# mcahny/vps

Measured on NVIDIA H100. Metric: FuseTrack frame pairs/s on synthetic 1024x2048 pairs, higher is better.
Workload: dtype f32 (wgmma: 3 split-f16 products per MAC, fp32 accumulate promoted to RN register sums)

## Files before the change

include/vps_b200.h:

```cpp
#ifndef VPS_B200_H_
#define VPS_B200_H_

#include <stdint.h>

#ifdef __cplusplus
extern "C" {
#endif

#define VPS_OK 0
#define VPS_E_ARG (-1)
#define VPS_E_CUDA (-2)
#define VPS_E_NODEV (-3)

#define VPS_F32 0
#define VPS_BF16 1

#define VPS_ACT_NONE 0
#define VPS_ACT_RELU 1
#define VPS_ACT_LRELU 2
#define VPS_ACT_SIGMOID 3

typedef struct vps_tensor {
  void* ptr;
  int32_t n, h, w, c;
// ... 7 lines not shown
void vps_add_launch_count(int64_t n);

typedef struct vps_conv_args {
  vps_tensor x, y, res;
  const void* w;
  const float* bias;
  int32_t kh, kw, sh, sw, ph, pw;
  int32_t oh, ow;
  int32_t oy_mul, oy_off, ox_mul, ox_off;
  int32_t cin, cout;
  int32_t act;
  float slope;
  int32_t res_after_act;
  float out_scale;
  int32_t cin_gran;
} vps_conv_args;

int vps_conv2d_tc(const vps_conv_args* a, void* stream);
int vps_conv2d_tc_multi(const vps_conv_args* a, int nprob, void* stream);
int vps_conv2d_simt(const vps_conv_args* a, void* stream);
int vps_pack_weights_tc(const float* w_oihw, const float* scale, void* dst_bf16, int cout, int cin,
                        int kh, int kw, int transposed, int cin_gran, void* stream);
int vps_pack_weights_simt(const float* w_oihw, const float* scale, float* dst, int cout, int cin,
                          int kh, int kw, int transposed, void* stream);
int64_t vps_packed_tc_bytes(int cout, int cin, int kh, int kw, int cin_gran);

int vps_conv2d_tc32(const vps_conv_args* a, void* stream);
int vps_conv2d_tc32_multi(const vps_conv_args* a, int nprob, void* stream);
int vps_conv2d_tc32_plan(const vps_conv_args* a, int nprob, int* plan);
int vps_pack_weights_tc32(const float* w_oihw, const float* scale, void* dst, int cout, int cin, int kh, int kw,
                          int transposed, int prob, int nprob, void* stream);
int64_t vps_packed_tc32_bytes(int cout, int cin, int kh, int kw, int nprob);
int vps_tc32_overflow(int reset);
int vps_deform_conv_tc32(const vps_tensor* x, const vps_tensor* offset, const void* w, int cout, const vps_tensor* y,
                         void* stream);
int vps_deform_conv_tc32_plan(const vps_tensor* x, int cout, int* plan);

int vps_im2col(const vps_tensor* x, const vps_tensor* cols, int kh, int kw, int sh, int sw, int ph,
               int pw, void* stream);

int vps_correlation(const vps_tensor* f1, const vps_tensor* f2, const vps_tensor* out, int pad,
                    int max_disp, int stride1, int stride2, int act, float slope, void* stream);
int vps_correlation_tc(const vps_tensor* f1, const vps_tensor* f2, const vps_tensor* out, int pad,
                       int max_disp, int stride1, int stride2, int act, float slope, void* stream);
// ... 112 lines not shown
```

vps_b200/_lib.py:

```python
import ctypes as C
import os

_HERE = os.path.dirname(os.path.abspath(__file__))
LIB_PATH = os.path.join(_HERE, "lib", "libvps_b200.so")

VPS_F32, VPS_BF16 = 0, 1
ACT_NONE, ACT_RELU, ACT_LRELU, ACT_SIGMOID = 0, 1, 2, 3


class VpsTensor(C.Structure):
    _fields_ = [("ptr", C.c_void_p), ("n", C.c_int32), ("h", C.c_int32), ("w", C.c_int32),
                ("c", C.c_int32), ("cs", C.c_int32), ("dtype", C.c_int32)]


class VpsConvArgs(C.Structure):
    _fields_ = [("x", VpsTensor), ("y", VpsTensor), ("res", VpsTensor),
                ("w", C.c_void_p), ("bias", C.c_void_p),
                ("kh", C.c_int32), ("kw", C.c_int32), ("sh", C.c_int32), ("sw", C.c_int32),
                ("ph", C.c_int32), ("pw", C.c_int32),
                ("oh", C.c_int32), ("ow", C.c_int32),
                ("oy_mul", C.c_int32), ("oy_off", C.c_int32), ("ox_mul", C.c_int32), ("ox_off", C.c_int32),
                ("cin", C.c_int32), ("cout", C.c_int32),
                ("act", C.c_int32), ("slope", C.c_float), ("res_after_act", C.c_int32),
                ("out_scale", C.c_float), ("cin_gran", C.c_int32)]


class VpsError(RuntimeError):
    pass


_lib = None


def lib():
    global _lib
    if _lib is None:
        if not os.path.exists(LIB_PATH):
            raise VpsError(
                "libvps_b200.so not found at %s -- run `python -c 'import __graft_entry__ as g; g.build()'`; "
                "there is no CPU/PyTorch fallback for the product path" % LIB_PATH)
        _lib = C.CDLL(LIB_PATH)
        _lib.vps_last_error.restype = C.c_char_p
        _lib.vps_launch_count.restype = C.c_int64
        _lib.vps_packed_tc_bytes.restype = C.c_int64
        _lib.vps_packed_tc32_bytes.restype = C.c_int64
        _lib.vps_correlation_tc32_ws_bytes.restype = C.c_int64
        _lib.vps_unify_pan_ws_bytes.restype = C.c_int64
        _lib.vps_unify_pan_error_offset.restype = C.c_int64
        _lib.vps_tube_confusion_ws_bytes.restype = C.c_int64
        _lib.vps_tube_confusion_ws_bytes.argtypes = [C.c_int64]
        _lib.vps_add_launch_count.restype = None
        _lib.vps_add_launch_count.argtypes = [C.c_int64]
    return _lib


def check(status, what=""):
    if status != 0:
        raise VpsError("%s failed (%d): %s" % (what, status, lib().vps_last_error().decode()))


EXPORTS = [
    "vps_last_error", "vps_version", "vps_launch_count", "vps_add_launch_count",
    "vps_conv2d_tc", "vps_conv2d_tc_multi", "vps_conv2d_simt", "vps_pack_weights_tc", "vps_pack_weights_simt",
    "vps_packed_tc_bytes", "vps_im2col",
    "vps_conv2d_tc32", "vps_conv2d_tc32_multi", "vps_conv2d_tc32_plan", "vps_pack_weights_tc32", "vps_packed_tc32_bytes", "vps_tc32_overflow", "vps_deform_conv_tc32", "vps_deform_conv_tc32_plan",
    "vps_correlation", "vps_correlation_tc", "vps_correlation_simt", "vps_correlation_tc32", "vps_correlation_tc32_ws_bytes", "vps_resample2d", "vps_channelnorm", "vps_flownet_input", "vps_flownet_stage", "vps_flownet_cat3", "vps_flow_deconv",
    "vps_nchw_to_nhwc", "vps_nhwc_to_nchw", "vps_copy_scale", "vps_axpby",
    "vps_space_to_depth2", "vps_tap_gather3x3", "vps_preprocess_u8", "vps_resize_bilinear", "vps_resize_nearest", "vps_pool2d", "vps_groupnorm",
    "vps_bfp_gather", "vps_bfp_scatter", "vps_flow_warp", "vps_tcea_temporal", "vps_tcea_combine",
    "vps_deform_im2col", "vps_deform_conv_tc",
    "vps_roi_align", "vps_sort_desc", "vps_rpn_decode", "vps_nms", "vps_nms_batch", "vps_sigmoid_flat", "vps_gather_rows",
    "vps_maskroi_candidates", "vps_track_assign",
    "vps_rpn_finalize", "vps_maskroi_finalize", "vps_select_class", "vps_track_update", "vps_det_split",
    "vps_mask_removal", "vps_panoptic_fuse", "vps_unify_pan", "vps_unify_pan_ws_bytes", "vps_unify_pan_error", "vps_unify_pan_error_offset", "vps_tube_confusion", "vps_tube_confusion_ws_bytes", "vps_rgb_to_id", "vps_pan2ch_ids",
]
```

vps_b200/csrc/conv_tc32.cu:

```cuda
#include "conv_tc_common.cuh"

namespace {

constexpr int T32_CONV_WARPS = 3;
constexpr int T32_KC = 32;
constexpr int T32_MAX_N = 128;
constexpr int T32_WIDE_MAX_N = 64;
constexpr int t32_threads(int nwg) { return 128 * (nwg + 1); }
constexpr int T32_STAGE_SLOTS = 2;
constexpr int T32_PLANES = 2;

__device__ unsigned int g_tc32_overflow = 0;

struct Tc32Extra {
  int rows;
  int plane_bytes;
  int stage_bytes;
  int b_plane_bytes;
  int dcn;
  int dcn_split_n;
};

struct Dcn32Params {
  const float* x;
  const float* off;
  int x_cs, off_cs, H, W;
};
constexpr int dcn32_setup_bytes(int rows) { return 9 * rows * 32; }
constexpr int DCN32_THREADS = 512;
constexpr int DCN32_GATHER_WARPS = 7;
constexpr int DCN32_MAX_N = 128;
constexpr int DCN32_LO_REGS = 80, DCN32_HI_REGS = 176;
static_assert(128 * (2 * DCN32_LO_REGS + 2 * DCN32_HI_REGS) == DCN32_THREADS * (65536 / DCN32_THREADS),
              "the DCN register split must use exactly the launch allocation");
static_assert(DCN32_LO_REGS % 8 == 0 && DCN32_HI_REGS % 8 == 0 && DCN32_LO_REGS >= 24 && DCN32_HI_REGS <= 256,
// ... 45 lines not shown
          }
          if (++ss == T32_STAGE_SLOTS) { ss = 0; sphase ^= 1; }
        }
        mbar_wait(rg.bempty(bs), bphase ^ 1);
        if (elect_one()) {
          mbar_expect_tx(rg.bfull(bs), b_bytes);
          tma_load_5d(rg.b_base + bs * rg.b_bytes, tmB, rg.bfull(bs), cc * T32_KC, n0, tap, t.prob, 0);
        }
        if (++bs == p.b_stages) { bs = 0; bphase ^= 1; }
        if (++s == kw) { s = 0; ++r; }
      }
    }
  }
}

__device__ __forceinline__ void converter32(const ConvTcParams& p, const Tc32Extra& e, const Ring32& rg, int ctid, int nthreads) {
  const int ntaps = p.kh * p.kw;
  const int items_per_tile = p.cin_chunks * (p.halo ? 1 : ntaps);
  const int tasks = e.rows * 4;
  int ss = 0, as = 0;
  uint32_t sphase = 0, aphase = 0;
  bool over = false;
  for (int tile = blockIdx.x; tile < p.total_tiles; tile += gridDim.x) {
    for (int it = 0; it < items_per_tile; ++it) {
      mbar_wait(rg.sfull(ss), sphase);
      mbar_wait(rg.pempty(as), aphase ^ 1);
      const uint32_t src = rg.s_base + ss * rg.s_bytes;
      const uint32_t dst = rg.a_base + as * rg.a_bytes;
      for (int task = ctid; task < tasks; task += nthreads) {
        const int r = task >> 2, j = task & 3;
// ... 265 lines not shown
template <int NWG, bool TMA_EPI>
__global__ void __launch_bounds__(t32_threads(NWG), 1)
conv_igemm_tc32_kernel(const __grid_constant__ CUtensorMap tmA, const __grid_constant__ CUtensorMap tmB,
                       const __grid_constant__ CUtensorMap tmY, const __grid_constant__ CUtensorMap tmR, const ConvTcParams p,
                       const Tc32Extra e) {
  extern __shared__ __align__(1024) uint8_t smem_raw[];
  const uint32_t smem_base = (smem_u32(smem_raw) + 1023u) & ~1023u;
  Ring32 rg;
  rg.s_base = smem_base; rg.s_bytes = (uint32_t)e.stage_bytes;
  rg.a_base = rg.s_base + T32_STAGE_SLOTS * rg.s_bytes; rg.a_bytes = (uint32_t)T32_PLANES * (uint32_t)e.plane_bytes;
  rg.b_base = rg.a_base + (uint32_t)p.a_stages * rg.a_bytes; rg.b_bytes = (uint32_t)T32_PLANES * (uint32_t)e.b_plane_bytes;
  rg.e_base = rg.b_base + (uint32_t)p.b_stages * rg.b_bytes;
  rg.bias_base = rg.e_base + (TMA_EPI ? 64u * NWG * (uint32_t)p.block_n * 4u : 0u);
  rg.bar_base = rg.bias_base + (TMA_EPI ? (uint32_t)NWG * (uint32_t)p.block_n * 4u : 0u);
  const int warp = __shfl_sync(0xffffffffu, (int)threadIdx.x >> 5, 0);
  if (warp == 0) init_bars32(rg, 32 * T32_CONV_WARPS, 32 * T32_CONV_WARPS, NWG);
  if (threadIdx.x == 32) {
    asm volatile("prefetch.tensormap [%0];" ::"l"(&tmA) : "memory");
    asm volatile("prefetch.tensormap [%0];" ::"l"(&tmB) : "memory");
    if (TMA_EPI) {
      asm volatile("prefetch.tensormap [%0];" ::"l"(&tmY) : "memory");
      if (p.res) asm volatile("prefetch.tensormap [%0];" ::"l"(&tmR) : "memory");
    }
  }
  __syncthreads();
  asm volatile("griddepcontrol.wait;" ::: "memory");
  asm volatile("griddepcontrol.launch_dependents;" ::: "memory");
  if (warp == 0) producer32(p, e, rg, &tmA, &tmB);
  else if (warp < 4) converter32(p, e, rg, (int)threadIdx.x - 32, 32 * T32_CONV_WARPS);
  else consumer32_n<NWG, TMA_EPI>(p, e, rg, (warp - 4) >> 2, &tmY, &tmR);
}

__global__ void __launch_bounds__(DCN32_THREADS, 1)
dcn_igemm_tc32_kernel(const __grid_constant__ CUtensorMap tmB, const ConvTcParams p, const Tc32Extra e, const Dcn32Params d) {
  extern __shared__ __align__(1024) uint8_t smem_raw[];
  const uint32_t smem_base = (smem_u32(smem_raw) + 1023u) & ~1023u;
  Ring32 rg;
  rg.s_base = smem_base; rg.s_bytes = 0;
  rg.a_base = smem_base; rg.a_bytes = (uint32_t)T32_PLANES * (uint32_t)e.plane_bytes;
  rg.b_base = rg.a_base + (uint32_t)p.a_stages * rg.a_bytes; rg.b_bytes = (uint32_t)T32_PLANES * (uint32_t)e.b_plane_bytes;
  const uint32_t setup_base = rg.b_base + (uint32_t)p.b_stages * rg.b_bytes;
  rg.bar_base = setup_base + dcn32_setup_bytes(e.rows);
  const int warp = __shfl_sync(0xffffffffu, (int)threadIdx.x >> 5, 0);
  if (warp == 0) init_bars32(rg, (uint32_t)e.rows / 8u, 1, 2);
// ... 24 lines not shown
                                         unsigned short* __restrict__ bl, int cout, int cin, int kh, int kw, int cout_pad,
                                         int cin_pad, int transposed) {
  const int64_t total = (int64_t)cout_pad * kh * kw * cin_pad;
  bool over = false;
  for (int64_t i = blockIdx.x * (int64_t)blockDim.x + threadIdx.x; i < total; i += (int64_t)gridDim.x * blockDim.x) {
    const float v = packed_weight(src, scale, i, cout, cin, kh, kw, cin_pad, transposed);
    unsigned short h, l;
    split_f16(v, h, l);
    over = over || f16_over(v);
    bm[i] = h;
    bl[i] = l;
  }
  if (over) atomicAdd(&g_tc32_overflow, 1u);
}

inline int64_t plane_elems(int cout, int cin, int kh, int kw) {
  const int64_t cout_pad = (cout + 15) / 16 * 16, cin_pad = (cin + T32_KC - 1) / T32_KC * T32_KC;
  return cout_pad * kh * kw * cin_pad;
}

constexpr int T32_SMEM_BUDGET = 227 * 1024 - 1024 - T32_BAR_BYTES - 64;

struct Tc32Plan {
  int nwg;
  int block_n;
  int halo, tw, th, halo_w, halo_h;
  int rows, stage_bytes, plane_bytes, a_stages, a_side;
  int b_stages;
  int epi_tma;
};

bool tc32_epi_expressible(const vps_conv_args* a, int nprob) {
  if (nprob != 1 || a->oy_mul != 1 || a->ox_mul != 1 || a->y.dtype != VPS_F32) return false;
  const int64_t px = (int64_t)a->oy_off * a->y.w + a->ox_off;
  if ((((uintptr_t)a->y.ptr + px * a->y.cs * 4) & 15) || a->y.cs % 4) return false;
  if (a->res.ptr && (a->res.dtype != VPS_F32 || (((uintptr_t)a->res.ptr + px * a->res.cs * 4) & 15) || a->res.cs % 4))
    return false;
  return true;
}

Tc32Plan tc32_tile(const vps_conv_args* a, int nwg) {
  Tc32Plan g = {};
  g.nwg = nwg;
  const int px = 64 * nwg;
  g.halo = a->sh == 1 && a->sw == 1 && a->kh * a->kw > 1 && a->kh <= 8 && a->kw <= 8;
  g.tw = g.halo ? 8 : patch_tw(a->oh, a->ow, px, a->sh, a->sw);
  g.th = px / g.tw;
  g.halo_w = g.tw + a->kw - 1;
  g.halo_h = g.th + a->kh - 1;
  g.rows = g.halo ? g.halo_h * g.halo_w : px;
  g.stage_bytes = (g.rows * 128 + 1023) / 1024 * 1024;
  g.plane_bytes = (g.rows * 64 + 1023) / 1024 * 1024;
  g.a_stages = g.halo ? 2 : 3;
  g.a_side = T32_STAGE_SLOTS * g.stage_bytes + g.a_stages * T32_PLANES * g.plane_bytes;
  return g;
}

int tc32_plan(const vps_conv_args* a, int nprob, Tc32Plan& out) {
  VPS_CHECK_ARG(nprob >= 1 && nprob <= MAX_PROB, "conv2d_tc32: nprob %d", nprob);
  VPS_CHECK_ARG(a->sh >= 1 && a->sh <= 2 && a->sw >= 1 && a->sw <= 2, "conv2d_tc32: stride must be 1 or 2");
  VPS_CHECK_ARG(a->kh >= 1 && a->kw >= 1 && a->cin >= 1 && a->cout >= 1 && a->oh >= 0 && a->ow >= 0 && a->x.n >= 0,
                "conv2d_tc32: bad geometry (k %dx%d, cin %d, cout %d, out %dx%d)", a->kh, a->kw, a->cin, a->cout, a->oh, a->ow);
  const int sms = vps::num_sms();
  if (sms <= 0) { vps::set_error("no device"); return VPS_E_NODEV; }
  const int cout_pad = (a->cout + 15) / 16 * 16;
  const int steps = (a->cin + T32_KC - 1) / T32_KC * a->kh * a->kw;
  double best = -1.0;
  for (int nwg = 2; nwg <= 4; nwg += 2) {
    Tc32Plan g = tc32_tile(a, nwg);
    const int64_t m_tiles = (int64_t)a->x.n * vps::cdiv(a->oh, g.th) * vps::cdiv(a->ow, g.tw) * nprob;
// ... 4 lines not shown
      const int64_t tiles = m_tiles * (cout_pad / bn);
      const double waves = (double)((tiles + sms - 1) / sms);
      const double step = fmax(fmax(300.0, 1.5 * nwg * bn), fmax((double)(bn * 64 * T32_PLANES) / 56.0, conv));
      const double t = waves * ((double)steps * step + 40.0 * bn + 1500.0);
      if (best < 0 || t < best * 0.999) {
        best = t;
        out = g;
        out.block_n = bn;
      }
    }
  }
  if (best < 0) {
    vps::set_error("conv2d_tc32: ring does not fit (k %dx%d)", a->kh, a->kw);
    return VPS_E_ARG;
  }
  const int eb = t32_epi_bytes(out.nwg, out.block_n), b2 = 2 * T32_PLANES * out.block_n * 64;
  out.epi_tma = 0;
  if (!out.halo && out.block_n <= T32_EPI_MAX_N && tc32_epi_expressible(a, nprob)) {
    if (out.a_side + b2 + eb > T32_SMEM_BUDGET && out.a_stages == 3 &&
        out.a_side - T32_PLANES * out.plane_bytes + b2 + eb <= T32_SMEM_BUDGET) {
      out.a_stages = 2;
      out.a_side -= T32_PLANES * out.plane_bytes;
    }
    out.epi_tma = out.a_side + b2 + eb <= T32_SMEM_BUDGET;
  }
  const int bst = (T32_SMEM_BUDGET - out.a_side - (out.epi_tma ? eb : 0)) / (T32_PLANES * out.block_n * 64);
  out.b_stages = bst > MAX_STAGES ? MAX_STAGES : bst;
  return VPS_OK;
}

// ... 40 lines not shown
    }
  }
  if (best < 0) {
    vps::set_error("deform_conv_tc32: no tiling fits (cout %d)", cout);
    return VPS_E_ARG;
  }
  return VPS_OK;
}

}

extern "C" int64_t vps_packed_tc32_bytes(int cout, int cin, int kh, int kw, int nprob) {
  return plane_elems(cout, cin, kh, kw) * 2 * T32_PLANES * nprob;
}

extern "C" unsigned int* vps_tc32_overflow_flag() {
  unsigned int* p = nullptr;
  if (cudaGetSymbolAddress((void**)&p, g_tc32_overflow) != cudaSuccess) return nullptr;
  return p;
}

extern "C" int vps_tc32_overflow(int reset) {
  unsigned int v = 0;
  if (cudaMemcpyFromSymbol(&v, g_tc32_overflow, sizeof(v)) != cudaSuccess) return -1;
  if (reset && v) {
    const unsigned int z = 0;
    cudaMemcpyToSymbol(g_tc32_overflow, &z, sizeof(z));
  }
  return (int)v;
}

extern "C" int vps_pack_weights_tc32(const float* w, const float* scale, void* dst, int cout, int cin, int kh, int kw,
                                     int transposed, int prob, int nprob, void* stream) {
  VPS_CHECK_ARG(nprob >= 1 && nprob <= MAX_PROB && prob >= 0 && prob < nprob, "pack_weights_tc32: prob %d of %d", prob, nprob);
// ... 28 lines not shown
  if (st != VPS_OK) return st;
  VPS_CHECK_ARG(g.b_stages >= 2, "conv2d_tc32: ring does not fit (%d x %d px halo, bn %d)", g.halo_h, g.halo_w, g.block_n);
  ConvTcParams p = {};
  Tc32Extra e = {};
  p.bk = T32_KC;
  const int cin_pad = (a->cin + T32_KC - 1) / T32_KC * T32_KC;
  const int cout_pad = (a->cout + 15) / 16 * 16;
  p.n_img = a->x.n; p.oh = a->oh; p.ow = a->ow;
  const bool halo = g.halo != 0;
  p.halo = g.halo;
  p.tw = g.tw; p.th = g.th;
  p.halo_w = g.halo_w;
  const int halo_h = g.halo_h;
  e.rows = g.rows;
  p.a_box_bytes = e.rows * 128;
  e.stage_bytes = g.stage_bytes;
  e.plane_bytes = g.plane_bytes;
  p.a_stage_bytes = T32_PLANES * e.plane_bytes;
  p.tiles_x = vps::cdiv(a->ow, p.tw); p.tiles_y = vps::cdiv(a->oh, p.th);
  p.kh = a->kh; p.kw = a->kw; p.sh = a->sh; p.sw = a->sw;
  p.cin_chunks = cin_pad / T32_KC;
  const int rem = a->cin - (p.cin_chunks - 1) * T32_KC;
  p.nk_last = (rem + 15) / 16;
  const int ntaps = a->kh * a->kw;
  p.a_stages = g.a_stages;
  const int block_n = g.block_n;
  p.block_n = block_n; p.n_tiles_n = cout_pad / block_n;
  e.b_plane_bytes = block_n * 64;
  p.b_stages = g.b_stages;
  p.nprob = nprob;
  p.tiles_per_prob = p.n_img * p.tiles_y * p.tiles_x * p.n_tiles_n;
  p.total_tiles = p.tiles_per_prob * nprob;
  st = set_problems(p, args, nprob, "conv2d_tc32");
  if (st != VPS_OK) return st;
  if (p.total_tiles == 0) return VPS_OK;

  CUtensorMap tmA, tmB;
  if (!vps::encode_nhwc(&tmA, a->x, CU_TENSOR_MAP_DATA_TYPE_FLOAT32, T32_KC, halo ? p.halo_w : p.tw * a->sw,
                        halo ? halo_h : p.th * a->sh, a->sw, a->sh, CU_TENSOR_MAP_SWIZZLE_128B, CU_TENSOR_MAP_L2_PROMOTION_L2_128B,
                        "conv2d_tc32: encode A"))
    return VPS_E_CUDA;
  const int64_t n_plane = (int64_t)cout_pad * ntaps * cin_pad;
  {
    cuuint64_t dims[5] = {(cuuint64_t)cin_pad, (cuuint64_t)cout_pad, (cuuint64_t)ntaps, (cuuint64_t)nprob, T32_PLANES};
    cuuint64_t strides[4] = {(cuuint64_t)ntaps * cin_pad * 2, (cuuint64_t)cin_pad * 2, (cuuint64_t)n_plane * 2,
                             (cuuint64_t)n_plane * nprob * 2};
    cuuint32_t box[5] = {(cuuint32_t)T32_KC, (cuuint32_t)block_n, 1, 1, T32_PLANES};
    cuuint32_t estr[5] = {1, 1, 1, 1, 1};
    CUresult r = encode(&tmB, CU_TENSOR_MAP_DATA_TYPE_UINT16, 5, (void*)a->w, dims, strides, box, estr, CU_TENSOR_MAP_INTERLEAVE_NONE,
                        CU_TENSOR_MAP_SWIZZLE_64B, CU_TENSOR_MAP_L2_PROMOTION_L2_256B, CU_TENSOR_MAP_FLOAT_OOB_FILL_NONE);
    if (r != CUDA_SUCCESS) { vps::set_error("conv2d_tc32: encode B failed (%d)", (int)r); return VPS_E_CUDA; }
  }
  CUtensorMap tmY = {}, tmR = {};
  if (g.epi_tma) {
    const int bc = t32_box_c(block_n), box_w = p.tw < 64 ? p.tw : 64;
    const int64_t px = (int64_t)a->oy_off * a->y.w + a->ox_off;
    for (int m = 0; m < (a->res.ptr ? 2 : 1); ++m) {
      const vps_tensor& t = m ? a->res : a->y;
      vps_tensor v = t;
      v.ptr = (float*)t.ptr + px * t.cs; v.n = a->x.n; v.h = a->oh; v.w = a->ow; v.c = a->cout;
      if (!vps::encode_nhwc(m ? &tmR : &tmY, v, CU_TENSOR_MAP_DATA_TYPE_FLOAT32, bc, box_w, 64 / box_w, 1, 1,
                            bc == 32 ? CU_TENSOR_MAP_SWIZZLE_128B : CU_TENSOR_MAP_SWIZZLE_64B, CU_TENSOR_MAP_L2_PROMOTION_L2_128B,
                            m ? "conv2d_tc32: encode residual" : "conv2d_tc32: encode output", &t))
        return VPS_E_CUDA;
    }
  }
  const int smem = g.a_side + p.b_stages * T32_PLANES * e.b_plane_bytes + (g.epi_tma ? t32_epi_bytes(g.nwg, block_n) : 0) + 1024 +
                   T32_BAR_BYTES;
#define VPS_TC32_LAUNCH(NWG, EPI)                                                                                              \
  launch_persistent<conv_igemm_tc32_kernel<NWG, EPI>>(p.total_tiles, t32_threads(NWG), smem, stream, "conv2d_tc32", tmA, tmB, tmY, \
                                                      tmR, p, e)
  if (g.nwg == 4) return g.epi_tma ? VPS_TC32_LAUNCH(4, true) : VPS_TC32_LAUNCH(4, false);
  return g.epi_tma ? VPS_TC32_LAUNCH(2, true) : VPS_TC32_LAUNCH(2, false);
#undef VPS_TC32_LAUNCH
}

extern "C" int vps_conv2d_tc32(const vps_conv_args* a, void* stream) { return vps_conv2d_tc32_multi(a, 1, stream); }

extern "C" int vps_conv2d_tc32_plan(const vps_conv_args* a, int nprob, int* plan) {
  Tc32Plan g;
  const int st = tc32_plan(a, nprob, g);
  if (st != VPS_OK) return st;
  plan[0] = g.nwg; plan[1] = g.block_n; plan[2] = g.tw; plan[3] = g.th; plan[4] = g.halo; plan[5] = g.epi_tma;
  return VPS_OK;
}


extern "C" int vps_deform_conv_tc32(const vps_tensor* x, const vps_tensor* offset, const void* w, int cout, const vps_tensor* y,
                                    void* stream) {
  VPS_CHECK_ARG(x->dtype == VPS_F32 && offset->dtype == VPS_F32 && offset->c >= 18, "deform_conv_tc32: dtypes");
  VPS_CHECK_ARG(x->c % T32_KC == 0 && x->cs % 8 == 0 && ((uintptr_t)x->ptr & 31) == 0,
                "deform_conv_tc32: x must have cin %% 32 == 0 and 32-byte aligned pixel rows (256-bit sampling loads)");
  VPS_CHECK_ARG(offset->n == x->n && offset->h == x->h && offset->w == x->w && y->n == x->n && y->h == x->h && y->w == x->w &&
                    y->c == cout, "deform_conv_tc32: shapes");
  VPS_CHECK_ARG((int64_t)x->n * x->h * x->w * x->cs < (1ll << 31), "deform_conv_tc32: tensor too large for 32-bit offsets");
  VPS_CHECK_ARG(((uintptr_t)w & 127) == 0, "deform_conv_tc32: weights not aligned");
  auto encode = vps::tensor_map_encoder();
  if (!encode) return VPS_E_CUDA;
  VPS_CHECK_ARG(y->dtype == VPS_F32, "deform_conv_tc32: y must be fp32");
// ... 56 lines not shown
```

vps_b200/csrc/corr_tc.cu:

```cuda
#include "conv_tc_common.cuh"

namespace {

constexpr int NPIX = 96;
constexpr int KC = 64;
constexpr int A_BYTES = 128 * KC * 2;
constexpr int B_BYTES = NPIX * KC * 2;
constexpr int A_STAGES = 6;
constexpr int MAX_KCH = 4;

struct CorrParams {
  int H, W, C, kch;
  int tiles_x, tiles_y, total_tiles;
  int n_img;
  void* out; int out_cs, out_dtype;
  int act; float slope;
  float scale;
  int accumulate;
  int f16;
};

template <int R, int S2, bool F16>
__device__ __forceinline__ void corr_consumer(const CorrParams& p, uint32_t a_ring, uint32_t b_buf, uint32_t bars, int wg) {
  constexpr int D = 2 * R + 1;
// ... 149 lines not shown
  static bool attr_set = false;
  if (!attr_set) {
    if (cudaFuncSetAttribute(kern, cudaFuncAttributeMaxDynamicSharedMemorySize, smem) != cudaSuccess) {
      vps::set_error("correlation_tc: smem attr: %s", cudaGetErrorString(cudaGetLastError()));
      return VPS_E_CUDA;
    }
    attr_set = true;
  }
  const int sms = vps::num_sms();
  const int grid = p.total_tiles < sms ? p.total_tiles : sms;
  kern<<<grid, 384, smem, st>>>(tm1, tm2, p);
  VPS_CUDA_LAST("corr_tc_kernel");
  return VPS_OK;
}

__global__ void split_f16_planes_kernel(const float* __restrict__ x, int64_t npix, int c, int cs, __half* __restrict__ hi,
                                        __half* __restrict__ lo, unsigned int* overflow) {
  const int64_t total = npix * (c / 4);
  bool over = false;
  for (int64_t i = blockIdx.x * (int64_t)blockDim.x + threadIdx.x; i < total; i += (int64_t)gridDim.x * blockDim.x) {
    const int64_t pix = i / (c / 4);
    const int c4 = (int)(i - pix * (c / 4)) * 4;
    const float4 v = *reinterpret_cast<const float4*>(x + pix * cs + c4);
    const float vv[4] = {v.x, v.y, v.z, v.w};
    __half h[4], l[4];
#pragma unroll
    for (int k = 0; k < 4; ++k) {
      unsigned short hb, lb;
      split_f16(vv[k], hb, lb);
      over = over || f16_over(vv[k]);
      h[k] = __ushort_as_half(hb); l[k] = __ushort_as_half(lb);
    }
    *reinterpret_cast<uint2*>(hi + pix * c + c4) = *reinterpret_cast<const uint2*>(h);
    *reinterpret_cast<uint2*>(lo + pix * c + c4) = *reinterpret_cast<const uint2*>(l);
  }
  if (over && overflow) atomicAdd(overflow, 1u);
}

}

extern "C" unsigned int* vps_tc32_overflow_flag();

extern "C" int64_t vps_correlation_tc32_ws_bytes(const vps_tensor* f1) {
  return 4 * (int64_t)f1->n * f1->h * f1->w * f1->c * 2 + 1024;
}

extern "C" int vps_correlation_tc32(const vps_tensor* f1, const vps_tensor* f2, const vps_tensor* out, int pad, int max_disp,
                                    int stride1, int stride2, int act, float slope, void* ws, void* stream) {
  VPS_CHECK_ARG(stride1 == 1 && pad == max_disp, "correlation_tc32: only stride1=1, pad==max_displacement");
  VPS_CHECK_ARG(f1->dtype == VPS_F32 && f2->dtype == VPS_F32 && out->dtype == VPS_F32, "correlation_tc32: fp32 tensors only");
  VPS_CHECK_ARG(f1->h == f2->h && f1->w == f2->w && f1->c == f2->c && f1->n == f2->n && out->h == f1->h && out->w == f1->w,
                "correlation_tc32: shape mismatch");
  VPS_CHECK_ARG(f1->c % KC == 0 && f1->c <= KC * MAX_KCH, "correlation_tc32: C must be a multiple of 64, <= 256");
  VPS_CHECK_ARG(f1->cs % 4 == 0 && f2->cs % 4 == 0 && ((uintptr_t)f1->ptr & 15) == 0 && ((uintptr_t)f2->ptr & 15) == 0 &&
                    ws && ((uintptr_t)ws & 255) == 0, "correlation_tc32: features / scratch must be aligned");
  VPS_CHECK_ARG(act == VPS_ACT_NONE || act == VPS_ACT_LRELU, "correlation_tc32: act");
  const int R = max_disp / stride2, D = 2 * R + 1;
  VPS_CHECK_ARG(out->c == D * D, "correlation_tc32: out.c %d != %d", out->c, D * D);
  VPS_CHECK_ARG((R == 10 && stride2 == 2) || (R == 4 && stride2 == 1), "correlation_tc32: unsupported (max_disp %d, stride2 %d)",
                max_disp, stride2);
  cudaStream_t st = (cudaStream_t)stream;
  const int64_t npix = (int64_t)f1->n * f1->h * f1->w, plane = npix * f1->c;
  __half* base = (__half*)ws;
  vps_tensor t[4];
  for (int i = 0; i < 4; ++i) {
    t[i] = *f1; t[i].ptr = base + i * plane; t[i].cs = f1->c; t[i].dtype = VPS_BF16;
  }
  unsigned int* flag = vps_tc32_overflow_flag();
  const int blocks = (int)((npix * (f1->c / 4) + 255) / 256 > 8192 ? 8192 : (npix * (f1->c / 4) + 255) / 256);
  split_f16_planes_kernel<<<blocks, 256, 0, st>>>((const float*)f1->ptr, npix, f1->c, f1->cs, base, base + plane, flag);
  VPS_CUDA_LAST("split_f16_planes");
  split_f16_planes_kernel<<<blocks, 256, 0, st>>>((const float*)f2->ptr, npix, f1->c, f2->cs, base + 2 * plane, base + 3 * plane, flag);
  VPS_CUDA_LAST("split_f16_planes");
  const float s1 = 1.0f / (float)f1->c, s2 = s1 * T32_LO_INV;
  int rc;
#define CORR_PASS(A, B, SC, ACC, ACT)                                                                        \
  rc = (R == 10) ? launch<10, 2>(&t[A], &t[B], out, ACT, slope, st, SC, ACC, 1) : launch<4, 1>(&t[A], &t[B], out, ACT, slope, st, SC, ACC, 1); \
  if (rc != VPS_OK) return rc;
  CORR_PASS(0, 2, s1, 0, VPS_ACT_NONE)
  CORR_PASS(0, 3, s2, 1, VPS_ACT_NONE)
  CORR_PASS(1, 2, s2, 1, act)
#undef CORR_PASS
  return VPS_OK;
}

extern "C" int vps_correlation_tc(const vps_tensor* f1, const vps_tensor* f2, const vps_tensor* out, int pad, int max_disp,
                                  int stride1, int stride2, int act, float slope, void* stream) {
  VPS_CHECK_ARG(stride1 == 1 && pad == max_disp, "correlation_tc: only stride1=1, pad==max_displacement");
  VPS_CHECK_ARG(f1->dtype == VPS_BF16 && f2->dtype == VPS_BF16, "correlation_tc: bf16 features only");
  VPS_CHECK_ARG(f1->h == f2->h && f1->w == f2->w && f1->c == f2->c && f1->n == f2->n && out->h == f1->h && out->w == f1->w,
// ... 14 lines not shown
```

vps_b200/ops.py:

```python
import ctypes as C
import os

import torch

from . import _lib
from ._lib import (ACT_LRELU, ACT_NONE, ACT_RELU, ACT_SIGMOID, VPS_BF16, VPS_F32, VpsConvArgs, VpsError,
                   VpsTensor, check, lib)

_DT = {torch.float32: VPS_F32, torch.bfloat16: VPS_BF16}

PROFILE = None
_NOTE = {"flops": 0, "tag": ""}
SCOPE = [""]
_real_lib = lib


class _ProfLib(object):
    def __getattr__(self, name):
        f = getattr(_real_lib(), name)
        if PROFILE is None or not name.startswith("vps_") or name in ("vps_last_error", "vps_launch_count", "vps_packed_tc_bytes"):
            return f

        def w(*a):
            s, e = torch.cuda.Event(enable_timing=True), torch.cuda.Event(enable_timing=True)
# ... 160 lines not shown
    kh, kw = pw.kh, pw.kw
    sh, sw = (stride, stride) if isinstance(stride, int) else stride
    ph, pw_ = pad_hw if pad_hw is not None else ((pad, pad) if isinstance(pad, int) else pad)
    a.kh, a.kw, a.sh, a.sw, a.ph, a.pw = kh, kw, sh, sw, ph, pw_
    if oh is None:
        oh = (x.shape[1] + 2 * ph - kh) // sh + 1
        ow = (x.shape[2] + 2 * pw_ - kw) // sw + 1
    a.oh, a.ow = oh, ow
    a.oy_mul, a.oy_off, a.ox_mul, a.ox_off = omap
    a.cin, a.cout = pw.cin, pw.cout
    a.act, a.slope, a.res_after_act, a.out_scale = act, slope, int(res_after_act), out_scale
    a.bias = pw.bias.data_ptr() if pw.bias is not None else None
    return a


def conv2d(x, pw, y, stride=1, pad=0, act=ACT_NONE, slope=0.1, res=None, res_after_act=False, out_scale=1.0,
           oh=None, ow=None, omap=(1, 0, 1, 0), pad_hw=None, use_tc=None):
    a = _conv_args(x, pw, y, stride, pad, act, slope, res, res_after_act, out_scale, oh, ow, omap, pad_hw)
    if use_tc is None:
        use_tc = x.dtype == torch.bfloat16
    if PROFILE is not None:
        _NOTE["flops"] = _NOTE.pop("flops_alg", None) or 2 * x.shape[0] * a.oh * a.ow * pw.cout * pw.cin * a.kh * a.kw
        _NOTE["tag"] = "%dx%d s%d %d->%d @%dx%d" % (a.kh, a.kw, a.sh, pw.cin, pw.cout, a.oh, a.ow)
    if use_tc and x.dtype == torch.float32:
        a.w = pw.tc32().data_ptr()
        check(lib().vps_conv2d_tc32(C.byref(a), stream()), "conv2d_tc32")
    elif use_tc:
        a.cin_gran = pw.gran()
        a.w = pw.tc().data_ptr()
        check(lib().vps_conv2d_tc(C.byref(a), stream()), "conv2d_tc")
    else:
        a.w = pw.simt().data_ptr()
        check(lib().vps_conv2d_simt(C.byref(a), stream()), "conv2d_simt")
    return y


def conv2d_tc_multi(x, pws, y, pads, omaps, act=ACT_NONE, slope=0.1, out_scale=1.0, oh=None, ow=None, shared32=None):
    n = len(pws)
    arr = (VpsConvArgs * n)()
    gran = pws[0].gran()
    f32 = x.dtype == torch.float32
    for i in range(n):
        a = _conv_args(x, pws[i], y, 1, 0, act, slope, None, False, out_scale, oh, ow, omaps[i], pads[i])
        a.cin_gran = gran
        a.w = shared32.data_ptr() if f32 else pws[i].tc(gran).data_ptr()
        arr[i] = a
    if PROFILE is not None:
        _NOTE["flops"] = 2 * x.shape[0] * arr[0].oh * arr[0].ow * pws[0].cout * pws[0].cin * arr[0].kh * arr[0].kw * n
        _NOTE["tag"] = "%dx%d x%d phases %d->%d @%dx%d" % (arr[0].kh, arr[0].kw, n, pws[0].cin, pws[0].cout, arr[0].oh, arr[0].ow)
    if f32:
        check(lib().vps_conv2d_tc32_multi(arr, n, stream()), "conv2d_tc32_multi")
    else:
        check(lib().vps_conv2d_tc_multi(arr, n, stream()), "conv2d_tc_multi")
    return y


def conv2d_tc32_plan(x, pws, stride=1, pad=0, oh=None, ow=None, pads=None, y=None, res=None, omaps=None):
    pws = pws if isinstance(pws, (list, tuple)) else [pws]
    n = len(pws)
    arr = (VpsConvArgs * n)()
    for i in range(n):
        arr[i] = _conv_args(x, pws[i], x if y is None else y, stride, pad, ACT_NONE, 0.1, res, False, 1.0, oh, ow,
                            omaps[i] if omaps is not None else (1, 0, 1, 0), pads[i] if pads is not None else None)
    plan = (C.c_int * 6)()
    check(_real_lib().vps_conv2d_tc32_plan(arr, n, plan), "conv2d_tc32_plan")
    return dict(nwg=plan[0], block_n=plan[1], tw=plan[2], th=plan[3], halo=plan[4], epilogue="tma" if plan[5] else "frag")


def correlation(f1, f2, out, pad, max_disp, stride1, stride2, act=ACT_NONE, slope=0.1, impl=None):
    fn = {None: "vps_correlation", "tc": "vps_correlation_tc", "simt": "vps_correlation_simt", "tc32": "vps_correlation_tc32"}[impl]
    if PROFILE is not None:
        d = 2 * (max_disp // stride2) + 1
        _NOTE["flops"] = 2 * f1.shape[0] * f1.shape[1] * f1.shape[2] * f1.shape[3] * d * d
        _NOTE["tag"] = "corr d%d s%d C%d @%dx%d" % (max_disp, stride2, f1.shape[3], f1.shape[1], f1.shape[2])
    if impl is None and F32_TC[0] and f1.dtype == torch.float32 and f2.dtype == torch.float32 and out.dtype == torch.float32:
        c = f1.shape[3]
        if (c % 64 == 0 and c <= 256 and stride1 == 1 and pad == max_disp and (max_disp, stride2) == (20, 2)
                and vt(f1).cs % 4 == 0 and vt(f2).cs % 4 == 0 and f1.data_ptr() % 16 == 0 and f2.data_ptr() % 16 == 0):
            fn = "vps_correlation_tc32"
    if fn == "vps_correlation_tc32":
        ws = torch.empty(int(lib().vps_correlation_tc32_ws_bytes(C.byref(vt(f1)))), dtype=torch.uint8, device=f1.device)
# ... 274 lines not shown
```

Before: 16.57.

## Add pre-split f16 feed path for tc32 convolutions chosen by cost model

Adds an optional feed mode for the fp32 tensor-core convolution. The input is split once into f16 hi/lo planes in a workspace by a separate kernel, and the producer then TMA-loads those planes directly, so the converter warps are bypassed. An auto cost model enables this when per-element conversion work inside the kernel, repeated across taps and N tiles, outweighs one extra split pass. The exchange is an extra kernel launch, workspace allocation and extra HBM traffic. The split kernel is now shared with correlation.

```diff
diff --git a/include/vps_b200.h b/include/vps_b200.h
--- a/include/vps_b200.h
+++ b/include/vps_b200.h
@@ -45,7 +45,12 @@
   int32_t res_after_act;
   float out_scale;
   int32_t cin_gran;
+  int32_t feed;
+  void* ws;
 } vps_conv_args;
+#define VPS_TC32_FEED_AUTO 0
+#define VPS_TC32_FEED_CONVERT 1
+#define VPS_TC32_FEED_PRESPLIT 2
 
 int vps_conv2d_tc(const vps_conv_args* a, void* stream);
 int vps_conv2d_tc_multi(const vps_conv_args* a, int nprob, void* stream);
@@ -59,6 +64,7 @@
 int vps_conv2d_tc32(const vps_conv_args* a, void* stream);
 int vps_conv2d_tc32_multi(const vps_conv_args* a, int nprob, void* stream);
 int vps_conv2d_tc32_plan(const vps_conv_args* a, int nprob, int* plan);
+int64_t vps_conv2d_tc32_ws_bytes(const vps_conv_args* a, int nprob);
 int vps_pack_weights_tc32(const float* w_oihw, const float* scale, void* dst, int cout, int cin, int kh, int kw,
                           int transposed, int prob, int nprob, void* stream);
 int64_t vps_packed_tc32_bytes(int cout, int cin, int kh, int kw, int nprob);
diff --git a/vps_b200/_lib.py b/vps_b200/_lib.py
--- a/vps_b200/_lib.py
+++ b/vps_b200/_lib.py
@@ -22,7 +22,10 @@
                 ("oy_mul", C.c_int32), ("oy_off", C.c_int32), ("ox_mul", C.c_int32), ("ox_off", C.c_int32),
                 ("cin", C.c_int32), ("cout", C.c_int32),
                 ("act", C.c_int32), ("slope", C.c_float), ("res_after_act", C.c_int32),
-                ("out_scale", C.c_float), ("cin_gran", C.c_int32)]
+                ("out_scale", C.c_float), ("cin_gran", C.c_int32), ("feed", C.c_int32), ("ws", C.c_void_p)]
+
+
+TC32_FEED = {None: 0, "convert": 1, "presplit": 2}
 
 
 class VpsError(RuntimeError):
@@ -45,6 +48,7 @@
         _lib.vps_packed_tc_bytes.restype = C.c_int64
         _lib.vps_packed_tc32_bytes.restype = C.c_int64
         _lib.vps_correlation_tc32_ws_bytes.restype = C.c_int64
+        _lib.vps_conv2d_tc32_ws_bytes.restype = C.c_int64
         _lib.vps_unify_pan_ws_bytes.restype = C.c_int64
         _lib.vps_unify_pan_error_offset.restype = C.c_int64
         _lib.vps_tube_confusion_ws_bytes.restype = C.c_int64
@@ -63,7 +67,7 @@
     "vps_last_error", "vps_version", "vps_launch_count", "vps_add_launch_count",
     "vps_conv2d_tc", "vps_conv2d_tc_multi", "vps_conv2d_simt", "vps_pack_weights_tc", "vps_pack_weights_simt",
     "vps_packed_tc_bytes", "vps_im2col",
-    "vps_conv2d_tc32", "vps_conv2d_tc32_multi", "vps_conv2d_tc32_plan", "vps_pack_weights_tc32", "vps_packed_tc32_bytes", "vps_tc32_overflow", "vps_deform_conv_tc32", "vps_deform_conv_tc32_plan",
+    "vps_conv2d_tc32", "vps_conv2d_tc32_multi", "vps_conv2d_tc32_plan", "vps_conv2d_tc32_ws_bytes", "vps_pack_weights_tc32", "vps_packed_tc32_bytes", "vps_tc32_overflow", "vps_deform_conv_tc32", "vps_deform_conv_tc32_plan",
     "vps_correlation", "vps_correlation_tc", "vps_correlation_simt", "vps_correlation_tc32", "vps_correlation_tc32_ws_bytes", "vps_resample2d", "vps_channelnorm", "vps_flownet_input", "vps_flownet_stage", "vps_flownet_cat3", "vps_flow_deconv",
     "vps_nchw_to_nhwc", "vps_nhwc_to_nchw", "vps_copy_scale", "vps_axpby",
     "vps_space_to_depth2", "vps_tap_gather3x3", "vps_preprocess_u8", "vps_resize_bilinear", "vps_resize_nearest", "vps_pool2d", "vps_groupnorm",
diff --git a/vps_b200/csrc/conv_tc32.cu b/vps_b200/csrc/conv_tc32.cu
--- a/vps_b200/csrc/conv_tc32.cu
+++ b/vps_b200/csrc/conv_tc32.cu
@@ -19,6 +19,7 @@
   int b_plane_bytes;
   int dcn;
   int dcn_split_n;
+  int presplit;
 };
 
 struct Dcn32Params {
@@ -94,6 +95,38 @@
   }
 }
 
+__device__ __forceinline__ void producer32_presplit(const ConvTcParams& p, const Ring32& rg, const CUtensorMap* tmA,
+                                                    const CUtensorMap* tmB, uint32_t b_bytes) {
+  const int ntaps = p.kh * p.kw, kw = p.kw;
+  const uint32_t a_box_bytes = (uint32_t)p.a_box_bytes;
+  int as = 0, bs = 0;
+  uint32_t aphase = 0, bphase = 0;
+  for (int tile = blockIdx.x; tile < p.total_tiles; tile += gridDim.x) {
+    const TileCoord t = tile_coord(p, tile);
+    const int x_base = t.tx * p.tw * p.sw - p.pw_[t.prob];
+    const int y_base = t.ty * p.th * p.sh - p.ph_[t.prob];
+    const int n0 = t.n_idx * p.block_n;
+    for (int cc = 0; cc < p.cin_chunks; ++cc) {
+      int r = 0, s = 0;
+      for (int tap = 0; tap < ntaps; ++tap) {
+        mbar_wait(rg.pempty(as), aphase ^ 1);
+        if (elect_one()) {
+          mbar_expect_tx(rg.pfull(as), a_box_bytes);
+          tma_load_5d(rg.a_base + as * rg.a_bytes, tmA, rg.pfull(as), cc * T32_KC, x_base + s, y_base + r, t.img, 0);
+        }
+        if (++as == p.a_stages) { as = 0; aphase ^= 1; }
+        mbar_wait(rg.bempty(bs), bphase ^ 1);
+        if (elect_one()) {
+          mbar_expect_tx(rg.bfull(bs), b_bytes);
+          tma_load_5d(rg.b_base + bs * rg.b_bytes, tmB, rg.bfull(bs), cc * T32_KC, n0, tap, t.prob, 0);
+        }
+        if (++bs == p.b_stages) { bs = 0; bphase ^= 1; }
+        if (++s == kw) { s = 0; ++r; }
+      }
+    }
+  }
+}
+
 __device__ __forceinline__ void converter32(const ConvTcParams& p, const Tc32Extra& e, const Ring32& rg, int ctid, int nthreads) {
   const int ntaps = p.kh * p.kw;
   const int items_per_tile = p.cin_chunks * (p.halo ? 1 : ntaps);
@@ -389,7 +422,7 @@
   rg.bias_base = rg.e_base + (TMA_EPI ? 64u * NWG * (uint32_t)p.block_n * 4u : 0u);
   rg.bar_base = rg.bias_base + (TMA_EPI ? (uint32_t)NWG * (uint32_t)p.block_n * 4u : 0u);
   const int warp = __shfl_sync(0xffffffffu, (int)threadIdx.x >> 5, 0);
-  if (warp == 0) init_bars32(rg, 32 * T32_CONV_WARPS, 32 * T32_CONV_WARPS, NWG);
+  if (warp == 0) init_bars32(rg, e.presplit ? 1 : 32 * T32_CONV_WARPS, 32 * T32_CONV_WARPS, NWG);
   if (threadIdx.x == 32) {
     asm volatile("prefetch.tensormap [%0];" ::"l"(&tmA) : "memory");
     asm volatile("prefetch.tensormap [%0];" ::"l"(&tmB) : "memory");
@@ -401,8 +434,11 @@
   __syncthreads();
   asm volatile("griddepcontrol.wait;" ::: "memory");
   asm volatile("griddepcontrol.launch_dependents;" ::: "memory");
-  if (warp == 0) producer32(p, e, rg, &tmA, &tmB);
-  else if (warp < 4) converter32(p, e, rg, (int)threadIdx.x - 32, 32 * T32_CONV_WARPS);
+  if (warp == 0 && e.presplit) producer32_presplit(p, rg, &tmA, &tmB, (uint32_t)T32_PLANES * (uint32_t)e.b_plane_bytes);
+  else if (warp == 0) producer32(p, e, rg, &tmA, &tmB);
+  else if (warp < 4) {
+    if (!e.presplit) converter32(p, e, rg, (int)threadIdx.x - 32, 32 * T32_CONV_WARPS);
+  }
   else consumer32_n<NWG, TMA_EPI>(p, e, rg, (warp - 4) >> 2, &tmY, &tmR);
 }
 
@@ -457,6 +493,37 @@
   if (over) atomicAdd(&g_tc32_overflow, 1u);
 }
 
+__global__ void split_f16_planes_kernel(const float* __restrict__ x, int64_t npix, int c, int cs, int c_pad,
+                                        uint4* __restrict__ hi, uint4* __restrict__ lo) {
+  const int chunks = c_pad / 8;
+  const int64_t total = npix * chunks;
+  bool over = false;
+  for (int64_t i = blockIdx.x * (int64_t)blockDim.x + threadIdx.x; i < total; i += (int64_t)gridDim.x * blockDim.x) {
+    const int64_t pix = i / chunks;
+    const int c0 = (int)(i - pix * chunks) * 8;
+    const float* src = x + pix * cs + c0;
+    float v[8];
+#pragma unroll
+    for (int q = 0; q < 2; ++q) {
+      if (c0 + 4 * q + 4 <= c) {
+        const float4 f = *reinterpret_cast<const float4*>(src + 4 * q);
+        v[4 * q] = f.x; v[4 * q + 1] = f.y; v[4 * q + 2] = f.z; v[4 * q + 3] = f.w;
+      } else {
+#pragma unroll
+        for (int k = 0; k < 4; ++k) v[4 * q + k] = c0 + 4 * q + k < c ? src[4 * q + k] : 0.f;
+      }
+    }
+    uint4 h, l;
+    split_pair_f16(v[0], v[1], h.x, l.x, over);
+    split_pair_f16(v[2], v[3], h.y, l.y, over);
+    split_pair_f16(v[4], v[5], h.z, l.z, over);
+    split_pair_f16(v[6], v[7], h.w, l.w, over);
+    hi[i] = h;
+    lo[i] = l;
+  }
+  if (over) atomicAdd(&g_tc32_overflow, 1u);
+}
+
 inline int64_t plane_elems(int cout, int cin, int kh, int kw) {
   const int64_t cout_pad = (cout + 15) / 16 * 16, cin_pad = (cin + T32_KC - 1) / T32_KC * T32_KC;
   return cout_pad * kh * kw * cin_pad;
@@ -471,6 +538,7 @@
   int rows, stage_bytes, plane_bytes, a_stages, a_side;
   int b_stages;
   int epi_tma;
+  int presplit;
 };
 
 bool tc32_epi_expressible(const vps_conv_args* a, int nprob) {
@@ -497,6 +565,39 @@
   g.a_stages = g.halo ? 2 : 3;
   g.a_side = T32_STAGE_SLOTS * g.stage_bytes + g.a_stages * T32_PLANES * g.plane_bytes;
   return g;
+}
+
+constexpr double T32_CONV_ITEM_CLK = 2000.0, T32_CONV_ROW_CLK = 6.0;
+constexpr double T32_FED_STEP_CLK = 950.0, T32_FED_MMA_CLK = 5.25;
+constexpr double T32_SPLIT_BYTES_PER_CLK = 1300.0;
+constexpr int T32_PRESPLIT_MIN_REUSE = 8;
+
+bool tc32_presplit_pays(const vps_conv_args* a, int nprob, const Tc32Plan& g, int sms) {
+  if (g.halo || nprob != 1 || a->oh == 0 || a->ow == 0 || a->kh < a->sh || a->kw < a->sw) return false;
+  if ((a->oh - 1) * a->sh - a->ph + a->kh < a->x.h || (a->ow - 1) * a->sw - a->pw + a->kw < a->x.w) return false;
+  const int cin_pad = (a->cin + T32_KC - 1) / T32_KC * T32_KC, cout_pad = (a->cout + 15) / 16 * 16;
+  if (a->kh * a->kw * (cout_pad / g.block_n) < T32_PRESPLIT_MIN_REUSE * a->sh * a->sw) return false;
+  const int64_t tiles = (int64_t)a->x.n * vps::cdiv(a->oh, g.th) * vps::cdiv(a->ow, g.tw) * (cout_pad / g.block_n);
+  const double waves = (double)((tiles + sms - 1) / sms);
+  const double steps = (double)(cin_pad / T32_KC) * a->kh * a->kw;
+  const double fed = T32_FED_STEP_CLK + T32_FED_MMA_CLK * g.nwg * g.block_n;
+  const double conv = fmax(fed, T32_CONV_ITEM_CLK + T32_CONV_ROW_CLK * g.rows);
+  const double split = 4.0 * (a->cin + cin_pad) * a->x.n * a->x.h * a->x.w / T32_SPLIT_BYTES_PER_CLK;
+  return waves * steps * (conv - fed) > split;
+}
+
+int tc32_presplit_rings(const vps_conv_args* a, Tc32Plan& g) {
+  const int a_slot = T32_PLANES * g.plane_bytes, b_slot = T32_PLANES * g.block_n * 64, eb = t32_epi_bytes(g.nwg, g.block_n);
+  VPS_CHECK_ARG(g.plane_bytes == g.rows * 64, "conv2d_tc32: pre-split A items of %d rows", g.rows);
+  g.stage_bytes = 0;
+  g.epi_tma = g.block_n <= T32_EPI_MAX_N && tc32_epi_expressible(a, 1) && 2 * (a_slot + b_slot) + eb <= T32_SMEM_BUDGET;
+  const int avail = T32_SMEM_BUDGET - (g.epi_tma ? eb : 0);
+  const int n = avail / (a_slot + b_slot);
+  g.a_stages = n > MAX_STAGES ? MAX_STAGES : n;
+  g.a_side = g.a_stages * a_slot;
+  const int bst = (avail - g.a_side) / b_slot;
+  g.b_stages = bst > MAX_STAGES ? MAX_STAGES : bst;
+  return VPS_OK;
 }
 
 int tc32_plan(const vps_conv_args* a, int nprob, Tc32Plan& out) {
@@ -531,6 +632,12 @@
     vps::set_error("conv2d_tc32: ring does not fit (k %dx%d)", a->kh, a->kw);
     return VPS_E_ARG;
   }
+  VPS_CHECK_ARG(a->feed >= VPS_TC32_FEED_AUTO && a->feed <= VPS_TC32_FEED_PRESPLIT, "conv2d_tc32: feed %d", a->feed);
+  VPS_CHECK_ARG(a->feed != VPS_TC32_FEED_PRESPLIT || (!out.halo && nprob == 1),
+                "conv2d_tc32: the pre-split feed needs flat tiles of one problem (k %dx%d, stride %d, %d problems)", a->kh, a->kw,
+                a->sh, nprob);
+  out.presplit = a->feed == VPS_TC32_FEED_PRESPLIT || (a->feed == VPS_TC32_FEED_AUTO && tc32_presplit_pays(a, nprob, out, sms));
+  if (out.presplit) return tc32_presplit_rings(a, out);
   const int eb = t32_epi_bytes(out.nwg, out.block_n), b2 = 2 * T32_PLANES * out.block_n * 64;
   out.epi_tma = 0;
   if (!out.halo && out.block_n <= T32_EPI_MAX_N && tc32_epi_expressible(a, nprob)) {
@@ -601,10 +708,17 @@
   return plane_elems(cout, cin, kh, kw) * 2 * T32_PLANES * nprob;
 }
 
-extern "C" unsigned int* vps_tc32_overflow_flag() {
-  unsigned int* p = nullptr;
-  if (cudaGetSymbolAddress((void**)&p, g_tc32_overflow) != cudaSuccess) return nullptr;
-  return p;
+extern "C" int vps_tc32_split_planes(const vps_tensor* x, int c_pad, void* hi, void* lo, void* stream) {
+  VPS_CHECK_ARG(x->dtype == VPS_F32 && x->cs % 4 == 0 && ((uintptr_t)x->ptr & 15) == 0 && c_pad >= x->c && c_pad % 8 == 0 &&
+                    ((uintptr_t)hi & 15) == 0 && ((uintptr_t)lo & 15) == 0,
+                "tc32_split_planes: x must be fp32 with 16-byte aligned pixels, c_pad %d >= c %d a multiple of 8", c_pad, x->c);
+  const int64_t npix = (int64_t)x->n * x->h * x->w, tasks = npix * (c_pad / 8);
+  if (tasks == 0) return VPS_OK;
+  const int blocks = (int)((tasks + 255) / 256 > 8192 ? 8192 : (tasks + 255) / 256);
+  split_f16_planes_kernel<<<blocks, 256, 0, (cudaStream_t)stream>>>((const float*)x->ptr, npix, x->c, x->cs, c_pad, (uint4*)hi,
+                                                                     (uint4*)lo);
+  VPS_CUDA_LAST("tc32_split_planes");
+  return VPS_OK;
 }
 
 extern "C" int vps_tc32_overflow(int reset) {
@@ -663,6 +777,7 @@
   const int halo_h = g.halo_h;
   e.rows = g.rows;
   p.a_box_bytes = e.rows * 128;
+  e.presplit = g.presplit;
   e.stage_bytes = g.stage_bytes;
   e.plane_bytes = g.plane_bytes;
   p.a_stage_bytes = T32_PLANES * e.plane_bytes;
@@ -685,10 +800,23 @@
   if (p.total_tiles == 0) return VPS_OK;
 
   CUtensorMap tmA, tmB;
-  if (!vps::encode_nhwc(&tmA, a->x, CU_TENSOR_MAP_DATA_TYPE_FLOAT32, T32_KC, halo ? p.halo_w : p.tw * a->sw,
-                        halo ? halo_h : p.th * a->sh, a->sw, a->sh, CU_TENSOR_MAP_SWIZZLE_128B, CU_TENSOR_MAP_L2_PROMOTION_L2_128B,
-                        "conv2d_tc32: encode A"))
+  const int64_t a_plane = (int64_t)a->x.n * a->x.h * a->x.w * cin_pad;
+  if (g.presplit) {
+    VPS_CHECK_ARG(a->ws && ((uintptr_t)a->ws & 255) == 0, "conv2d_tc32: the pre-split feed needs vps_conv2d_tc32_ws_bytes() of "
+                  "256-byte aligned workspace");
+    cuuint64_t dims[5] = {(cuuint64_t)cin_pad, (cuuint64_t)a->x.w, (cuuint64_t)a->x.h, (cuuint64_t)a->x.n, T32_PLANES};
+    cuuint64_t strides[4] = {(cuuint64_t)cin_pad * 2, (cuuint64_t)a->x.w * cin_pad * 2, (cuuint64_t)a->x.h * a->x.w * cin_pad * 2,
+                             (cuuint64_t)a_plane * 2};
+    cuuint32_t box[5] = {(cuuint32_t)T32_KC, (cuuint32_t)(p.tw * a->sw), (cuuint32_t)(p.th * a->sh), 1, T32_PLANES};
+    cuuint32_t estr[5] = {1, (cuuint32_t)a->sw, (cuuint32_t)a->sh, 1, 1};
+    CUresult r = encode(&tmA, CU_TENSOR_MAP_DATA_TYPE_FLOAT16, 5, a->ws, dims, strides, box, estr, CU_TENSOR_MAP_INTERLEAVE_NONE,
+                        CU_TENSOR_MAP_SWIZZLE_64B, CU_TENSOR_MAP_L2_PROMOTION_L2_128B, CU_TENSOR_MAP_FLOAT_OOB_FILL_NONE);
+    if (r != CUDA_SUCCESS) { vps::set_error("conv2d_tc32: encode pre-split A failed (%d)", (int)r); return VPS_E_CUDA; }
+  } else if (!vps::encode_nhwc(&tmA, a->x, CU_TENSOR_MAP_DATA_TYPE_FLOAT32, T32_KC, halo ? p.halo_w : p.tw * a->sw,
+                               halo ? halo_h : p.th * a->sh, a->sw, a->sh, CU_TENSOR_MAP_SWIZZLE_128B,
+                               CU_TENSOR_MAP_L2_PROMOTION_L2_128B, "conv2d_tc32: encode A")) {
     return VPS_E_CUDA;
+  }
   const int64_t n_plane = (int64_t)cout_pad * ntaps * cin_pad;
   {
     cuuint64_t dims[5] = {(cuuint64_t)cin_pad, (cuuint64_t)cout_pad, (cuuint64_t)ntaps, (cuuint64_t)nprob, T32_PLANES};
@@ -716,6 +844,10 @@
   }
   const int smem = g.a_side + p.b_stages * T32_PLANES * e.b_plane_bytes + (g.epi_tma ? t32_epi_bytes(g.nwg, block_n) : 0) + 1024 +
                    T32_BAR_BYTES;
+  if (g.presplit) {
+    st = vps_tc32_split_planes(&a->x, cin_pad, a->ws, (uint16_t*)a->ws + a_plane, stream);
+    if (st != VPS_OK) return st;
+  }
 #define VPS_TC32_LAUNCH(NWG, EPI)                                                                                              \
   launch_persistent<conv_igemm_tc32_kernel<NWG, EPI>>(p.total_tiles, t32_threads(NWG), smem, stream, "conv2d_tc32", tmA, tmB, tmY, \
                                                       tmR, p, e)
@@ -731,7 +863,15 @@
   const int st = tc32_plan(a, nprob, g);
   if (st != VPS_OK) return st;
   plan[0] = g.nwg; plan[1] = g.block_n; plan[2] = g.tw; plan[3] = g.th; plan[4] = g.halo; plan[5] = g.epi_tma;
+  plan[6] = g.presplit ? VPS_TC32_FEED_PRESPLIT : VPS_TC32_FEED_CONVERT;
   return VPS_OK;
+}
+
+extern "C" int64_t vps_conv2d_tc32_ws_bytes(const vps_conv_args* a, int nprob) {
+  Tc32Plan g;
+  if (tc32_plan(a, nprob, g) != VPS_OK) return -1;
+  const int64_t cin_pad = (a->cin + T32_KC - 1) / T32_KC * T32_KC;
+  return g.presplit ? (int64_t)T32_PLANES * 2 * a->x.n * a->x.h * a->x.w * cin_pad : 0;
 }
 
 
diff --git a/vps_b200/csrc/corr_tc.cu b/vps_b200/csrc/corr_tc.cu
--- a/vps_b200/csrc/corr_tc.cu
+++ b/vps_b200/csrc/corr_tc.cu
@@ -187,32 +187,9 @@
   return VPS_OK;
 }
 
-__global__ void split_f16_planes_kernel(const float* __restrict__ x, int64_t npix, int c, int cs, __half* __restrict__ hi,
-                                        __half* __restrict__ lo, unsigned int* overflow) {
-  const int64_t total = npix * (c / 4);
-  bool over = false;
-  for (int64_t i = blockIdx.x * (int64_t)blockDim.x + threadIdx.x; i < total; i += (int64_t)gridDim.x * blockDim.x) {
-    const int64_t pix = i / (c / 4);
-    const int c4 = (int)(i - pix * (c / 4)) * 4;
-    const float4 v = *reinterpret_cast<const float4*>(x + pix * cs + c4);
-    const float vv[4] = {v.x, v.y, v.z, v.w};
-    __half h[4], l[4];
-#pragma unroll
-    for (int k = 0; k < 4; ++k) {
-      unsigned short hb, lb;
-      split_f16(vv[k], hb, lb);
-      over = over || f16_over(vv[k]);
-      h[k] = __ushort_as_half(hb); l[k] = __ushort_as_half(lb);
-    }
-    *reinterpret_cast<uint2*>(hi + pix * c + c4) = *reinterpret_cast<const uint2*>(h);
-    *reinterpret_cast<uint2*>(lo + pix * c + c4) = *reinterpret_cast<const uint2*>(l);
-  }
-  if (over && overflow) atomicAdd(overflow, 1u);
-}
-
-}
-
-extern "C" unsigned int* vps_tc32_overflow_flag();
+}
+
+extern "C" int vps_tc32_split_planes(const vps_tensor* x, int c_pad, void* hi, void* lo, void* stream);
 
 extern "C" int64_t vps_correlation_tc32_ws_bytes(const vps_tensor* f1) {
   return 4 * (int64_t)f1->n * f1->h * f1->w * f1->c * 2 + 1024;
@@ -239,14 +216,11 @@
   for (int i = 0; i < 4; ++i) {
     t[i] = *f1; t[i].ptr = base + i * plane; t[i].cs = f1->c; t[i].dtype = VPS_BF16;
   }
-  unsigned int* flag = vps_tc32_overflow_flag();
-  const int blocks = (int)((npix * (f1->c / 4) + 255) / 256 > 8192 ? 8192 : (npix * (f1->c / 4) + 255) / 256);
-  split_f16_planes_kernel<<<blocks, 256, 0, st>>>((const float*)f1->ptr, npix, f1->c, f1->cs, base, base + plane, flag);
-  VPS_CUDA_LAST("split_f16_planes");
-  split_f16_planes_kernel<<<blocks, 256, 0, st>>>((const float*)f2->ptr, npix, f1->c, f2->cs, base + 2 * plane, base + 3 * plane, flag);
-  VPS_CUDA_LAST("split_f16_planes");
+  int rc = vps_tc32_split_planes(f1, f1->c, base, base + plane, stream);
+  if (rc != VPS_OK) return rc;
+  rc = vps_tc32_split_planes(f2, f1->c, base + 2 * plane, base + 3 * plane, stream);
+  if (rc != VPS_OK) return rc;
   const float s1 = 1.0f / (float)f1->c, s2 = s1 * T32_LO_INV;
-  int rc;
 #define CORR_PASS(A, B, SC, ACC, ACT)                                                                        \
   rc = (R == 10) ? launch<10, 2>(&t[A], &t[B], out, ACT, slope, st, SC, ACC, 1) : launch<4, 1>(&t[A], &t[B], out, ACT, slope, st, SC, ACC, 1); \
   if (rc != VPS_OK) return rc;
diff --git a/vps_b200/ops.py b/vps_b200/ops.py
--- a/vps_b200/ops.py
+++ b/vps_b200/ops.py
@@ -198,9 +198,19 @@
     return a
 
 
+def _tc32_ws(arr, n, device):
+    nbytes = int(_real_lib().vps_conv2d_tc32_ws_bytes(arr, n))
+    if nbytes < 0:
+        check(-1, "conv2d_tc32_ws_bytes")
+    ws = torch.empty(nbytes, dtype=torch.uint8, device=device) if nbytes else None
+    arr[0].ws = ws.data_ptr() if ws is not None else None
+    return ws
+
+
 def conv2d(x, pw, y, stride=1, pad=0, act=ACT_NONE, slope=0.1, res=None, res_after_act=False, out_scale=1.0,
-           oh=None, ow=None, omap=(1, 0, 1, 0), pad_hw=None, use_tc=None):
+           oh=None, ow=None, omap=(1, 0, 1, 0), pad_hw=None, use_tc=None, feed=None):
     a = _conv_args(x, pw, y, stride, pad, act, slope, res, res_after_act, out_scale, oh, ow, omap, pad_hw)
+    a.feed = _lib.TC32_FEED[feed]
     if use_tc is None:
         use_tc = x.dtype == torch.bfloat16
     if PROFILE is not None:
@@ -208,6 +218,7 @@
         _NOTE["tag"] = "%dx%d s%d %d->%d @%dx%d" % (a.kh, a.kw, a.sh, pw.cin, pw.cout, a.oh, a.ow)
     if use_tc and x.dtype == torch.float32:
         a.w = pw.tc32().data_ptr()
+        ws = _tc32_ws(C.pointer(a), 1, x.device)
         check(lib().vps_conv2d_tc32(C.byref(a), stream()), "conv2d_tc32")
     elif use_tc:
         a.cin_gran = pw.gran()
@@ -233,22 +244,25 @@
         _NOTE["flops"] = 2 * x.shape[0] * arr[0].oh * arr[0].ow * pws[0].cout * pws[0].cin * arr[0].kh * arr[0].kw * n
         _NOTE["tag"] = "%dx%d x%d phases %d->%d @%dx%d" % (arr[0].kh, arr[0].kw, n, pws[0].cin, pws[0].cout, arr[0].oh, arr[0].ow)
     if f32:
+        ws = _tc32_ws(arr, n, x.device)
         check(lib().vps_conv2d_tc32_multi(arr, n, stream()), "conv2d_tc32_multi")
     else:
         check(lib().vps_conv2d_tc_multi(arr, n, stream()), "conv2d_tc_multi")
     return y
 
 
-def conv2d_tc32_plan(x, pws, stride=1, pad=0, oh=None, ow=None, pads=None, y=None, res=None, omaps=None):
+def conv2d_tc32_plan(x, pws, stride=1, pad=0, oh=None, ow=None, pads=None, y=None, res=None, omaps=None, feed=None):
     pws = pws if isinstance(pws, (list, tuple)) else [pws]
     n = len(pws)
     arr = (VpsConvArgs * n)()
     for i in range(n):
         arr[i] = _conv_args(x, pws[i], x if y is None else y, stride, pad, ACT_NONE, 0.1, res, False, 1.0, oh, ow,
                             omaps[i] if omaps is not None else (1, 0, 1, 0), pads[i] if pads is not None else None)
-    plan = (C.c_int * 6)()
+    arr[0].feed = _lib.TC32_FEED[feed]
+    plan = (C.c_int * 7)()
     check(_real_lib().vps_conv2d_tc32_plan(arr, n, plan), "conv2d_tc32_plan")
-    return dict(nwg=plan[0], block_n=plan[1], tw=plan[2], th=plan[3], halo=plan[4], epilogue="tma" if plan[5] else "frag")
+    return dict(nwg=plan[0], block_n=plan[1], tw=plan[2], th=plan[3], halo=plan[4], epilogue="tma" if plan[5] else "frag",
+                feed="presplit" if plan[6] == _lib.TC32_FEED["presplit"] else "convert")
 
 
 def correlation(f1, f2, out, pad, max_disp, stride1, stride2, act=ACT_NONE, slope=0.1, impl=None):
```

Measured after the change: 16.99 (median of 6 runs). +2.5%, better.
